# VISION-SJTU/UniDefense

Hardware: AMD Instinct MI355X
Metric: images/sec fwd+bwd (256x256, EffNet-b4) (higher is better)
Workload: dtype f32

## Files before the change

### unidefense_amd/csrc/gemm_p3.hip

```cpp
#include "gemm_internal.h"
#include "ud_common.h"

#include <algorithm>
#include <type_traits>

namespace {

constexpr int NT = 512;
constexpr int BK = 32;
constexpr int BM = 128, BN = 128;
constexpr int PLANE_IMG = 128 * 64;

template <int PREC> struct Cfg {
    static constexpr int NPL = PREC;
    static constexpr int OP_IMG = NPL * PLANE_IMG;
    static constexpr int STAGE = 2 * OP_IMG;
    static constexpr int NSTAGE = PREC == 3 ? 3 : 4;
    static constexpr int PT = 4 * NPL;
    static constexpr int NTERM = PREC == 3 ? 6 : PREC == 2 ? 3 : 1;
};

typedef __bf16 bf16x8 __attribute__((ext_vector_type(8)));
typedef _Float16 f16x8 __attribute__((ext_vector_type(8)));
typedef short s16x4 __attribute__((ext_vector_type(4)));
// ... 294 lines not shown
                    for (int r = 0; r < 16; ++r) {
                        const double v = (double)acc[i][j][r];
                        s1 += v;
                        s2 += v * v;
                    }
                s1 += __shfl_xor(s1, 32, 64);
                s2 += __shfl_xor(s2, 32, 64);
                const int col = n0 + wn * 64 + j * 32 + l31;
                if (half == 0 && col < dN) {
                    unsafeAtomicAdd(stat_sum + slot + col, s1);
                    unsafeAtomicAdd(stat_sumsq + slot + col, s2);
                }
            }
        }
        auto store_all = [&](auto mode_c, auto inside_c) {
            constexpr int MODE = decltype(mode_c)::value;
            constexpr bool INSIDE = decltype(inside_c)::value;
#pragma unroll
            for (int i = 0; i < 2; ++i) {
#pragma unroll
                for (int j = 0; j < 2; ++j) {
                    const int col = n0 + wn * 64 + j * 32 + l31;
                    const long off0 = (long)(m0 + wm * 64 + i * 32 + 4 * half) * ldc + col;
                    float* pc = Cp + off0;
#pragma unroll
                    for (int r = 0; r < 16; ++r) {
                        const int dr = (r & 3) + 8 * (r >> 2);
                        if (INSIDE || (m0 + wm * 64 + i * 32 + 4 * half + dr < dM && col < dN)) {
                            const float v = acc[i][j][r];
                            if constexpr (MODE >= 4) {
                                _Float16* p = reinterpret_cast<_Float16*>(Cp) + off0 + (long)dr * ldc;
                                *p = (_Float16)(MODE == 4 ? v : v + (float)*p);
                            } else {
                                float* p = pc + (long)dr * ldc;
                                if constexpr (MODE == 0) *p = v;
                                else if constexpr (MODE == 1) *p += v;
                                else atomicAdd(p, v);
                            }
                        }
                    }
                }
            }
        };
        const bool inside = m0 + BM <= dM && n0 + BN <= dN;
        if (PREC == 1 && c_half) {
            if (inside) {
                if (ep == 0) store_all(integral_constant<int, 4>{}, T{});
                else store_all(integral_constant<int, 5>{}, T{});
            } else {
                if (ep == 0) store_all(integral_constant<int, 4>{}, F{});
                else store_all(integral_constant<int, 5>{}, F{});
            }
        } else if (inside) {
            if (ep == 0) store_all(integral_constant<int, 0>{}, T{});
            else if (ep == 1) store_all(integral_constant<int, 1>{}, T{});
            else store_all(integral_constant<int, 2>{}, T{});
        } else {
            if (ep == 0) store_all(integral_constant<int, 0>{}, F{});
            else if (ep == 1) store_all(integral_constant<int, 1>{}, F{});
            else store_all(integral_constant<int, 2>{}, F{});
        }
    };

    if constexpr (!SK) {
        int tile_m = bx % tiles_m, tile_n = bx / tiles_m;
        if (d.tile_cfg & 0x200) {
            const int GM = (d.tile_cfg >> 12) & 15 ? (d.tile_cfg >> 12) & 15 : 4;
            const int Tn = tiles_m * tiles_n, q = Tn >> 3, r = Tn & 7, x = bx & 7;
            const int o = x * q + (x < r ? x : r) + (bx >> 3);
            const int per_group = GM * tiles_n, g = o / per_group, first_m = g * GM;
            const int gm = min(GM, tiles_m - first_m), in = o - g * per_group;
            tile_n = in / gm;
            tile_m = first_m + in - tile_n * gm;
        }
        const int split = by;
        const int kt_per = (kt_total + d.split_k - 1) / d.split_k;
        const int kt0 = split * kt_per;
        const int nkt = min(kt_per, kt_total - kt0);
        segment(tile_m, tile_n, kt0, nkt, d.out_mode == 3 ? 0 : d.out_mode,
                d.C + (d.out_mode == 3 ? (long)split * d.slice_stride : 0L), true);
    } else {
        const int G = gx, b = bx;
        const int g = (b & 7) * (G >> 3) + (b >> 3);
        const long U = (long)tiles_m * tiles_n * kt_total;
        long u = g * U / G;
        const long u1 = (g + 1) * U / G;
        const int band_tiles = 8 * tiles_m;
        bool first = true;
        while (u < u1) {
            const int tile = (int)(u / kt_total), kt_b = (int)(u - (long)tile * kt_total);
            const int kt_e = (int)min((long)kt_total, kt_b + (u1 - u));
            const int band = tile / band_tiles, in_band = tile - band * band_tiles;
            const int bw = min(8, tiles_n - band * 8);
            const int tile_m = in_band / bw, tile_n = band * 8 + in_band - tile_m * bw;
            const bool whole = kt_b == 0 && kt_e == kt_total;
            segment(tile_m, tile_n, kt_b, kt_e - kt_b, whole ? d.out_mode : 2, d.C, first);
            first = false;
            u += kt_e - kt_b;
        }
    }
}

template <int PREC, int AMODE, int BMODE, bool SK = false>
__global__ __launch_bounds__(NT, 1) void gemm_p3_kernel(const ud_gemm_p3_desc d, int tiles_m, int tiles_n) {
    using CF = Cfg<PREC>;
    __shared__ __attribute__((aligned(1024))) char L[CF::NSTAGE * CF::STAGE];
    p3_body<PREC, AMODE, BMODE, SK>(d, tiles_m, tiles_n, L, (int)blockIdx.x, (int)blockIdx.y, (int)gridDim.x);
}

template <int PREC, int A0 = 0, int B0 = 1, int A1 = 1, int B1 = 1>
__global__ __launch_bounds__(NT, 1) void gemm_p3_pair_kernel(const ud_gemm_p3_desc d0, int tm0, int tn0, int n0,
                                                              const ud_gemm_p3_desc d1, int tm1, int tn1) {
    using CF = Cfg<PREC>;
    __shared__ __attribute__((aligned(1024))) char L[CF::NSTAGE * CF::STAGE];
    const int b = (int)blockIdx.x;
    const bool first = b < (n0 < 0 ? -n0 : n0);
    const int l = first ? b : b - (n0 < 0 ? -n0 : n0);
    if (first == (n0 > 0)) {
        const int T = tm0 * tn0;
        p3_body<PREC, A0, B0, false>(d0, tm0, tn0, L, l % T, l / T, T);
    } else {
        const int T = tm1 * tn1;
        p3_body<PREC, A1, B1, false>(d1, tm1, tn1, L, l % T, l / T, T);
    }
}

int num_cus() {
    static const int n = [] {
        int dev = 0, cus = 0;
        if (hipGetDevice(&dev) != hipSuccess ||
            hipDeviceGetAttribute(&cus, hipDeviceAttributeMultiprocessorCount, dev) != hipSuccess || cus < 8)
            cus = 256;
        return cus;
    }();
    return n;
}

template <int PREC, int AMODE, int BMODE>
int launch(const ud_gemm_p3_desc& d, hipStream_t s) {
    const int tiles_m = ud_cdiv(d.M, BM), tiles_n = ud_cdiv(d.N, BN);
    if (d.tile_cfg & 0x800) {
        const long U = (long)tiles_m * tiles_n * (d.K / BK);
        long G = std::min<long>(num_cus(), U / 4);
        G = std::max<long>(8, G / 8 * 8);
        hipLaunchKernelGGL((gemm_p3_kernel<PREC, AMODE, BMODE, true>), dim3((unsigned)G), dim3(NT), 0, s, d, tiles_m, tiles_n);
    } else {
        dim3 grid((unsigned)(tiles_m * tiles_n), (unsigned)d.split_k, 1);
        hipLaunchKernelGGL((gemm_p3_kernel<PREC, AMODE, BMODE>), grid, dim3(NT), 0, s, d, tiles_m, tiles_n);
    }
    UD_LAUNCH_CHECK();
    return 0;
}

__device__ __forceinline__ uint32_t pack_bf16(float x, float y) {
    typedef __bf16 bf16x2 __attribute__((ext_vector_type(2)));
    bf16x2 v = {(__bf16)x, (__bf16)y};
    return __builtin_bit_cast(uint32_t, v);
}
__device__ __forceinline__ void split2(float x, float y, uint32_t& p0, uint32_t& p1, uint32_t& p2) {
    p0 = pack_bf16(x, y);
    const float rx = x - __uint_as_float(p0 << 16), ry = y - __uint_as_float(p0 & 0xffff0000u);
    p1 = pack_bf16(rx, ry);
    const float sx = rx - __uint_as_float(p1 << 16), sy = ry - __uint_as_float(p1 & 0xffff0000u);
    p2 = pack_bf16(sx, sy);
}

typedef uint32_t u32x4 __attribute__((ext_vector_type(4)));
typedef uint32_t u32x2 __attribute__((ext_vector_type(2)));

__global__ __launch_bounds__(256) void split_planes_kernel(const float* __restrict__ x, long R, int C, long ld,
                                                           uint16_t* __restrict__ out, long panel, long plane) {
    const int tid = threadIdx.x;
    const long row = (long)blockIdx.x * 64 + (tid >> 2);
    const int pan = blockIdx.y, c0 = pan * 32 + (tid & 3) * 8;
    if (row >= R) return;
    f32x4 v0 = {0.f, 0.f, 0.f, 0.f}, v1 = {0.f, 0.f, 0.f, 0.f};
    if (c0 + 8 <= C) {
        v0 = *reinterpret_cast<const f32x4*>(x + row * ld + c0);
        v1 = *reinterpret_cast<const f32x4*>(x + row * ld + c0 + 4);
    } else if (c0 + 4 <= C) {
        v0 = *reinterpret_cast<const f32x4*>(x + row * ld + c0);
    }
    uint32_t a[4], b[4], c[4];
    split2(v0[0], v0[1], a[0], b[0], c[0]);
    split2(v0[2], v0[3], a[1], b[1], c[1]);
    split2(v1[0], v1[1], a[2], b[2], c[2]);
    split2(v1[2], v1[3], a[3], b[3], c[3]);
    const u32x4 p0 = {a[0], a[1], a[2], a[3]}, p1 = {b[0], b[1], b[2], b[3]}, p2 = {c[0], c[1], c[2], c[3]};
    uint16_t* o = out + (long)pan * panel + row * 32 + (tid & 3) * 8;
    *reinterpret_cast<u32x4*>(o) = p0;
    *reinterpret_cast<u32x4*>(o + plane) = p1;
    *reinterpret_cast<u32x4*>(o + 2 * plane) = p2;
}

typedef _Float16 f16x2 __attribute__((ext_vector_type(2)));
__device__ __forceinline__ void split2h(float x, float y, uint32_t& h0, uint32_t& h1) {
    const f16x2 a = {(_Float16)x, (_Float16)y};
    h0 = __builtin_bit_cast(uint32_t, a);
    const f16x2 b = {(_Float16)((x - (float)a[0]) * 2048.f), (_Float16)((y - (float)a[1]) * 2048.f)};
    h1 = __builtin_bit_cast(uint32_t, b);
}

constexpr int H2_MAXQ = 16;

__global__ __launch_bounds__(256) void split_h2_rows_kernel(const float* __restrict__ x, long R, int C, long ld,
                                                            uint16_t* __restrict__ out, long panel, long plane,
                                                            float* __restrict__ inv_scale) {
    const int lane = threadIdx.x & 63;
    const long row = (long)blockIdx.x * 4 + (threadIdx.x >> 6);
    if (row >= R) return;
    const int nq = C >> 2;
    const f32x4* xr = reinterpret_cast<const f32x4*>(x + row * ld);
    f32x4 v[H2_MAXQ];
    float m = 0.f;
#pragma unroll
    for (int i = 0; i < H2_MAXQ; ++i) {
        const int q = lane + 64 * i;
        v[i] = q < nq ? xr[q] : f32x4{0.f, 0.f, 0.f, 0.f};
        m = fmaxf(m, fmaxf(fmaxf(fabsf(v[i][0]), fabsf(v[i][1])), fmaxf(fabsf(v[i][2]), fabsf(v[i][3]))));
    }
    m = ud_wave_max(m);
    const int e = (int)(__float_as_uint(m) >> 23) & 0xff;
    int fs = m > 0.f ? 268 - e : 127;
    fs = fs < 1 ? 1 : fs > 254 ? 254 : fs;
    const float s = __uint_as_float((uint32_t)fs << 23), inv = __uint_as_float((uint32_t)(254 - fs) << 23);
    if (lane == 0) inv_scale[row] = inv;
    const int nq_pad = ((C + 31) >> 5) << 3;
#pragma unroll
    for (int i = 0; i < H2_MAXQ; ++i) {
        const int q = lane + 64 * i;
        if (q < nq_pad) {
            uint32_t a0, a1, b0, b1;
            split2h(v[i][0] * s, v[i][1] * s, a0, a1);
            split2h(v[i][2] * s, v[i][3] * s, b0, b1);
            uint16_t* o = out + (long)(q >> 3) * panel + row * 32 + (q & 7) * 4;
            *reinterpret_cast<u32x2*>(o) = u32x2{a0, b0};
            *reinterpret_cast<u32x2*>(o + plane) = u32x2{a1, b1};
        }
    }
}

constexpr int ABSMAX_SLOTS = 256;
__global__ __launch_bounds__(1024) void absmax_kernel(const float* __restrict__ x, long R, int C, long ld, uint32_t* __restrict__ out) {
    __shared__ float red[16];
    const long nq = R * (long)(C >> 2);
    const int cq = C >> 2;
    const long stride = (long)ABSMAX_SLOTS * 1024;
    float m = 0.f;
    auto at = [&](long q) {
        const long r = q / cq;
        return *reinterpret_cast<const f32x4*>(x + r * ld + (q - r * cq) * 4);
    };
    long q = (long)blockIdx.x * 1024 + threadIdx.x;
    for (; q + stride < nq; q += 2 * stride) {
        const f32x4 v = at(q), w = at(q + stride);
        m = fmaxf(m, fmaxf(fmaxf(fabsf(v[0]), fabsf(v[1])), fmaxf(fabsf(v[2]), fabsf(v[3]))));
        m = fmaxf(m, fmaxf(fmaxf(fabsf(w[0]), fabsf(w[1])), fmaxf(fabsf(w[2]), fabsf(w[3]))));
    }
    if (q < nq) {
        const f32x4 v = at(q);
        m = fmaxf(m, fmaxf(fmaxf(fabsf(v[0]), fabsf(v[1])), fmaxf(fabsf(v[2]), fabsf(v[3]))));
    }
    m = ud_wave_max(m);
    if ((threadIdx.x & 63) == 0) red[threadIdx.x >> 6] = m;
    __syncthreads();
    if (threadIdx.x == 0) {
        float t = red[0];
#pragma unroll
        for (int i = 1; i < 16; ++i) t = fmaxf(t, red[i]);
        out[blockIdx.x] = __float_as_uint(t);
    }
}

__device__ __forceinline__ void h2_scale(uint32_t bits, float& s, float& inv) { ud_h2_scale(bits, s, inv); }

__global__ __launch_bounds__(256) void split_h2_tensor_kernel(const float* __restrict__ x, long R, int C, long ld,
                                                              uint16_t* __restrict__ out, long panel, long plane,
                                                              const uint32_t* __restrict__ absmax, float* __restrict__ inv_scale) {
    const int tid = threadIdx.x;
    const long row = (long)blockIdx.x * 64 + (tid >> 2);
    const int pan = blockIdx.y, c0 = pan * 32 + (tid & 3) * 8;
    uint32_t mb = 0;
#pragma unroll
    for (int i = 0; i < ABSMAX_SLOTS / 64; ++i) mb = max(mb, absmax[(tid & 63) + 64 * i]);
#pragma unroll
    for (int o = 32; o > 0; o >>= 1) mb = max(mb, (uint32_t)__shfl_xor((int)mb, o, 64));
    float s, inv;
    h2_scale(mb, s, inv);
    if (blockIdx.x == 0 && blockIdx.y == 0 && tid == 0) *inv_scale = inv;
    if (row >= R) return;
    f32x4 v0 = {0.f, 0.f, 0.f, 0.f}, v1 = {0.f, 0.f, 0.f, 0.f};
    if (c0 + 8 <= C) {
        v0 = *reinterpret_cast<const f32x4*>(x + row * ld + c0);
        v1 = *reinterpret_cast<const f32x4*>(x + row * ld + c0 + 4);
    } else if (c0 + 4 <= C) {
        v0 = *reinterpret_cast<const f32x4*>(x + row * ld + c0);
    }
    uint32_t a[4], b[4];
    split2h(v0[0] * s, v0[1] * s, a[0], b[0]);
    split2h(v0[2] * s, v0[3] * s, a[1], b[1]);
    split2h(v1[0] * s, v1[1] * s, a[2], b[2]);
    split2h(v1[2] * s, v1[3] * s, a[3], b[3]);
    uint16_t* o = out + (long)pan * panel + row * 32 + (tid & 3) * 8;
    *reinterpret_cast<u32x4*>(o) = u32x4{a[0], a[1], a[2], a[3]};
    *reinterpret_cast<u32x4*>(o + plane) = u32x4{b[0], b[1], b[2], b[3]};
}
// ... 102 lines not shown
    float m = 0.f;
    for (long q = (long)bl * 1024 + threadIdx.x; q < nq; q += stride) {
        const long r = q / cq;
        const f32x4 v = *reinterpret_cast<const f32x4*>(it.x + r * it.ld + (q - r * cq) * 4);
        m = fmaxf(m, fmaxf(fmaxf(fabsf(v[0]), fabsf(v[1])), fmaxf(fabsf(v[2]), fabsf(v[3]))));
    }
    m = ud_wave_max(m);
    if ((threadIdx.x & 63) == 0) red[threadIdx.x >> 6] = m;
    __syncthreads();
    if (threadIdx.x == 0) {
        float t = red[0];
#pragma unroll
        for (int k = 1; k < 16; ++k) t = fmaxf(t, red[k]);
        slots[(long)i * ABSMAX_SLOTS + bl] = __float_as_uint(t);
    }
}

__global__ __launch_bounds__(256) void split_h2_multi_kernel(const ud_split_item* __restrict__ items, int n,
                                                             const uint32_t* __restrict__ slots) {
    const int i = item_of_block(items, n, blockIdx.x, true);
    const ud_split_item it = items[i];
    const int bl = blockIdx.x - it.split_block0;
    const int pan = bl / it.split_bx, bx = bl - pan * it.split_bx;
    const int tid = threadIdx.x;
    const long row = (long)bx * 64 + (tid >> 2);
    const int c0 = pan * 32 + (tid & 3) * 8;
    const uint32_t* absmax = slots + (long)i * ABSMAX_SLOTS;
    uint32_t mb = 0;
#pragma unroll
    for (int k = 0; k < ABSMAX_SLOTS / 64; ++k) mb = max(mb, absmax[(tid & 63) + 64 * k]);
#pragma unroll
    for (int o = 32; o > 0; o >>= 1) mb = max(mb, (uint32_t)__shfl_xor((int)mb, o, 64));
    float s, inv;
    h2_scale(mb, s, inv);
    if (bl == 0 && tid == 0) *it.inv_scale = inv;
    if (row >= it.R) return;
    f32x4 v0 = {0.f, 0.f, 0.f, 0.f}, v1 = {0.f, 0.f, 0.f, 0.f};
    if (c0 + 8 <= it.C) {
        v0 = *reinterpret_cast<const f32x4*>(it.x + row * it.ld + c0);
        v1 = *reinterpret_cast<const f32x4*>(it.x + row * it.ld + c0 + 4);
    } else if (c0 + 4 <= it.C) {
        v0 = *reinterpret_cast<const f32x4*>(it.x + row * it.ld + c0);
    }
    uint32_t a[4], b[4];
    split2h(v0[0] * s, v0[1] * s, a[0], b[0]);
    split2h(v0[2] * s, v0[3] * s, a[1], b[1]);
    split2h(v1[0] * s, v1[1] * s, a[2], b[2]);
    split2h(v1[2] * s, v1[3] * s, a[3], b[3]);
    uint16_t* o = it.out + (long)pan * it.panel + row * 32 + (tid & 3) * 8;
    *reinterpret_cast<u32x4*>(o) = u32x4{a[0], a[1], a[2], a[3]};
    *reinterpret_cast<u32x4*>(o + it.plane) = u32x4{b[0], b[1], b[2], b[3]};
}

}

extern "C" int ud_split_planes_h2t_multi(const ud_split_item* items_dev, int n, uint32_t* slots, int amax_blocks_total,
                                         int split_blocks_total, ud_stream_t stream) {
    if (!items_dev || !slots || n < 1 || amax_blocks_total < n || split_blocks_total < n) return UD_EINVAL;
    hipStream_t s = (hipStream_t)stream;
    hipLaunchKernelGGL(absmax_multi_kernel, dim3((unsigned)amax_blocks_total), dim3(1024), 0, s, items_dev, n, slots);
    hipLaunchKernelGGL(split_h2_multi_kernel, dim3((unsigned)split_blocks_total), dim3(256), 0, s, items_dev, n, slots);
    UD_LAUNCH_CHECK();
    return 0;
}

extern "C" int ud_im2col_planes(const float* x, const ud_conv_geom* g, uint16_t* planes, long panel_stride, long plane_stride,
                                const uint32_t* absmax, float* inv_scale, ud_stream_t stream) {
    if (!x || !g || !planes || !absmax || !inv_scale || g->transposed || g->Cin < 32 || g->Cin % 32 || g->N < 1 || g->Hin < 1 ||
        g->Win < 1 || g->Hout < 1 || g->Wout < 1 || g->KH < 1 || g->KW < 1 || g->stride < 1)
        return UD_EINVAL;
    const long M = (long)g->N * g->Hout * g->Wout, Kc = (long)g->KH * g->KW * g->Cin;
    if (panel_stride < M * 32 || panel_stride % 8 || plane_stride % 8 || plane_stride < (Kc / 32) * panel_stride) return UD_EINVAL;
    dim3 grid((unsigned)ud_cdiv(M, 64), (unsigned)(Kc / 32));
    hipLaunchKernelGGL(im2col_planes_kernel, grid, dim3(256), 0, (hipStream_t)stream, x, *g, planes, panel_stride, plane_stride,
                       absmax, inv_scale);
    UD_LAUNCH_CHECK();
    return 0;
}

extern "C" int ud_col2im(const float* dcol, const ud_conv_geom* g, float* dx, ud_stream_t stream) {
    if (!dcol || !g || !dx || g->transposed || g->Cin % 4 || g->stride < 1) return UD_EINVAL;
    const long total = (long)g->N * g->Hin * g->Win * (g->Cin / 4);
    long blocks = (total + 255) / 256;
    if (blocks > 16384) blocks = 16384;
    hipLaunchKernelGGL(col2im_kernel, dim3((unsigned)blocks), dim3(256), 0, (hipStream_t)stream, dcol, *g, dx);
    UD_LAUNCH_CHECK();
    return 0;
}

extern "C" int ud_absmax(const float* x, long R, int C, long ld, uint32_t* out, ud_stream_t stream) {
    if (!x || !out || R <= 0 || C <= 0 || C % 4 != 0 || ld % 4 != 0 || ld < C) return UD_EINVAL;
    hipLaunchKernelGGL(absmax_kernel, dim3(ABSMAX_SLOTS), dim3(1024), 0, (hipStream_t)stream, x, R, C, ld, out);
    UD_LAUNCH_CHECK();
    return 0;
}

extern "C" int ud_split_planes_h2t(const float* x, long R, int C, long ld, uint16_t* planes, long panel_stride,
                                   long plane_stride, const uint32_t* absmax, float* inv_scale, ud_stream_t stream) {
    if (!x || !planes || !absmax || !inv_scale || R <= 0 || C <= 0 || C % 4 != 0 || ld % 4 != 0 || ld < C ||
        panel_stride < R * 32 || panel_stride % 8 != 0 || plane_stride % 8 != 0 ||
        plane_stride < (long)ud_cdiv(C, 32) * panel_stride)
        return UD_EINVAL;
    dim3 grid((unsigned)ud_cdiv(R, 64), (unsigned)ud_cdiv(C, 32));
    hipLaunchKernelGGL(split_h2_tensor_kernel, grid, dim3(256), 0, (hipStream_t)stream, x, R, C, ld, planes, panel_stride,
                       plane_stride, absmax, inv_scale);
    UD_LAUNCH_CHECK();
    return 0;
}

extern "C" int ud_planes_from_half(const void* x, long R, int C, long ld, uint16_t* planes, long panel_stride, float* inv_scale,
                                   ud_stream_t stream) {
    if (!x || !planes || !inv_scale || R < 1 || C < 8 || C % 8 || ld < C || ld % 8 || panel_stride < 32 * R || panel_stride % 8 ||
        ((uintptr_t)x & 15))
        return UD_EINVAL;
    dim3 grid((unsigned)ud_cdiv(R, 64), (unsigned)ud_cdiv(C, 32));
    hipLaunchKernelGGL(planes_from_half_kernel, grid, dim3(256), 0, (hipStream_t)stream, (const uint16_t*)x, R, C, ld, planes,
                       panel_stride, inv_scale);
    UD_LAUNCH_CHECK();
    return 0;
}

extern "C" int ud_split_planes(const float* x, long R, int C, long ld, uint16_t* planes, long panel_stride,
                               long plane_stride, ud_stream_t stream) {
    if (!x || !planes || R <= 0 || C <= 0 || C % 4 != 0 || ld % 4 != 0 || ld < C || panel_stride < R * 32 ||
        panel_stride % 8 != 0 || plane_stride % 8 != 0 || plane_stride < (long)ud_cdiv(C, 32) * panel_stride)
        return UD_EINVAL;
    dim3 grid((unsigned)ud_cdiv(R, 64), (unsigned)ud_cdiv(C, 32));
    hipLaunchKernelGGL(split_planes_kernel, grid, dim3(256), 0, (hipStream_t)stream, x, R, C, ld, planes, panel_stride,
                       plane_stride);
    UD_LAUNCH_CHECK();
    return 0;
}

extern "C" int ud_split_planes_h2(const float* x, long R, int C, long ld, uint16_t* planes, long panel_stride,
                                  long plane_stride, float* inv_scale, ud_stream_t stream) {
    if (!x || !planes || !inv_scale || R <= 0 || C <= 0 || C % 4 != 0 || C > 256 * H2_MAXQ || ld % 4 != 0 || ld < C ||
        panel_stride < R * 32 || panel_stride % 8 != 0 || plane_stride % 8 != 0 ||
        plane_stride < (long)ud_cdiv(C, 32) * panel_stride)
        return UD_EINVAL;
    hipLaunchKernelGGL(split_h2_rows_kernel, dim3((unsigned)ud_cdiv(R, 4)), dim3(256), 0, (hipStream_t)stream, x, R, C, ld,
                       planes, panel_stride, plane_stride, inv_scale);
    UD_LAUNCH_CHECK();
    return 0;
}

static bool p3_desc_ok(const ud_gemm_p3_desc& d);

extern "C" int ud_gemm_p3_pair(const ud_gemm_p3_desc* nn, const ud_gemm_p3_desc* tn, ud_stream_t stream) {
    if (!nn || !tn || !p3_desc_ok(*nn) || !p3_desc_ok(*tn)) return UD_EINVAL;
    const ud_gemm_p3_desc &d0 = *nn, &d1 = *tn;
    const bool grads = d0.a_mode == 0 && d0.b_mode == 1 && d1.a_mode == 1 && d1.b_mode == 1;
    const bool tailp = d0.a_mode == 0 && d0.b_mode == 0 && d1.a_mode == 0 && d1.b_mode == 0 && d0.prec == 2;
    if ((d0.prec != 2 && d0.prec != 1) || d1.prec != d0.prec || !(grads || tailp)) return UD_EINVAL;
    if ((d0.tile_cfg | d1.tile_cfg) & 0x800) return UD_EINVAL;
    if (d0.stat_sum || d1.stat_sum || d0.out_mode == 3 || d1.out_mode == 3) return UD_EINVAL;
    const int tm0 = ud_cdiv(d0.M, BM), tn0 = ud_cdiv(d0.N, BN), tm1 = ud_cdiv(d1.M, BM), tn1 = ud_cdiv(d1.N, BN);
    const long n0 = (long)tm0 * tn0 * d0.split_k, n1 = (long)tm1 * tn1 * d1.split_k;
    if (n0 + n1 > 0x7fffffffL) return UD_EINVAL;
    const int nfirst = (d1.tile_cfg & 0x10000) ? -(int)n1 : (int)n0;
    if (tailp)
        hipLaunchKernelGGL((gemm_p3_pair_kernel<2, 0, 0, 0, 0>), dim3((unsigned)(n0 + n1)), dim3(NT), 0, (hipStream_t)stream, d0, tm0,
                           tn0, nfirst, d1, tm1, tn1);
    else if (d0.prec == 1)
        hipLaunchKernelGGL((gemm_p3_pair_kernel<1>), dim3((unsigned)(n0 + n1)), dim3(NT), 0, (hipStream_t)stream, d0, tm0, tn0,
                           nfirst, d1, tm1, tn1);
    else
        hipLaunchKernelGGL((gemm_p3_pair_kernel<2>), dim3((unsigned)(n0 + n1)), dim3(NT), 0, (hipStream_t)stream, d0, tm0, tn0,
                           nfirst, d1, tm1, tn1);
    UD_LAUNCH_CHECK();
    return 0;
}

static bool p3_desc_ok(const ud_gemm_p3_desc& d) {
    if (!d.A || !d.B || !d.C || d.M <= 0 || d.N <= 0 || d.K <= 0 || d.K % BK != 0 || d.split_k < 1 ||
        d.split_k > d.K / BK || d.out_mode < 0 || d.out_mode > 3 || d.a_mode < 0 || d.a_mode > 1 || d.b_mode < 0 ||
        d.b_mode > 1 || d.a_panel % 8 != 0 || d.b_panel % 8 != 0 || d.a_plane % 8 != 0 || d.b_plane % 8 != 0 ||
        d.a_npanel < 1 || d.b_npanel < 1 || d.prec < 1 || d.prec > 3)
        return false;
    if (d.prec <= 2 && (!d.a_inv_scale || !d.b_inv_scale || d.a_scale_stride < 0 || d.a_scale_stride > 1 ||
                        d.b_scale_stride < 0 || d.b_scale_stride > 1))
        return false;
    if (d.stat_sum && (d.out_mode != 0 || d.split_k != 1 || !d.stat_sumsq || (d.tile_cfg & 0x800))) return false;
    if ((d.tile_cfg & 0x800) && (d.out_mode > 1 || d.split_k != 1)) return false;
    if (d.out_mode == 3 && d.slice_stride < (long)d.M * d.ldc) return false;
    if (d.c_half && (d.prec != 1 || d.out_mode > 1 || d.split_k != 1 || (d.tile_cfg & 0x800))) return false;
    return true;
}

extern "C" int ud_gemm_p3(const ud_gemm_p3_desc* dp, ud_stream_t stream) {
    if (!dp) return UD_EINVAL;
    const ud_gemm_p3_desc& d = *dp;
    if (!p3_desc_ok(d)) return UD_EINVAL;
    hipStream_t s = (hipStream_t)stream;
    if (d.prec == 1) {
        if (d.a_mode == 0 && d.b_mode == 0) return launch<1, 0, 0>(d, s);
        if (d.a_mode == 0 && d.b_mode == 1) return launch<1, 0, 1>(d, s);
        if (d.a_mode == 1 && d.b_mode == 1) return launch<1, 1, 1>(d, s);
        return UD_EINVAL;
    }
    if (d.prec == 2) {
        if (d.a_mode == 0 && d.b_mode == 0) return launch<2, 0, 0>(d, s);
        if (d.a_mode == 0 && d.b_mode == 1) return launch<2, 0, 1>(d, s);
        if (d.a_mode == 1 && d.b_mode == 1) return launch<2, 1, 1>(d, s);
        return UD_EINVAL;
    }
    if (d.a_mode == 0 && d.b_mode == 0) return launch<3, 0, 0>(d, s);
    if (d.a_mode == 0 && d.b_mode == 1) return launch<3, 0, 1>(d, s);
    if (d.a_mode == 1 && d.b_mode == 1) return launch<3, 1, 1>(d, s);
    if (d.a_mode == 1 && d.b_mode == 0) return launch<3, 1, 0>(d, s);
    return UD_EINVAL;
}
```

### unidefense_amd/kernels.py

```python
import ctypes as C
import math
import os

import torch

from . import lib as _lib
from .config import cfg as CFG
from .devmem import Scratch, ZeroPool
from .lib import ConvGeom, GemmDesc, GemmP3Desc

_call = _lib.call
_const, _rows = _lib.const, _lib.const_rows

GEMM_PROFILE = None


def _stream():
    return C.c_void_p(torch.cuda.current_stream().cuda_stream)


def _p(t):
    if t is None:
        return None
    return C.c_void_p(t.data_ptr())
# ... 570 lines not shown
            e1.record()
        e1.synchronize()
        cur.wait_stream(s)
        return e0.elapsed_time(e1) / (2 * n)
    except Exception:
        torch.cuda.synchronize()
        e0.record()
        for _ in range(n):
            fn()
        e1.record()
        e1.synchronize()
        return e0.elapsed_time(e1) / n


def _tuned_plan(kind, M, N, K, launch, baseline, extra_if_split=None, no_split=False):
    kind = kind if isinstance(kind, str) else "/".join(str(v) for v in kind)
    key = (kind, M, N, K, extra_if_split is not None, _call("ud_gemm_get_path"))
    if key in _TUNED:
        return _TUNED[key]
    if not CFG.gemm_tune or torch.cuda.is_current_stream_capturing() or min(M, N, K) < _X3_MINDIM:
        return None
    best_t, best = _time_launches(baseline), None
    extra = _time_launches(extra_if_split) if extra_if_split is not None else 0.0
    for cfg, split in _tune_candidates(M, N, K):
        if no_split and split > 1:
            continue
        t = _time_launches(lambda: launch(cfg, split)) + (extra if split > 1 else 0.0)
        if t < 0.97 * best_t:
            best_t, best = t, (cfg, split)
    _TUNED[key] = best
    _tune_cache_save()
    return best


def _model_plan_launch(a, w, out, M, N, K, lda, ldb, b_mode, acc):
    plan = _tail_plan(M, N, K)
    if plan is not None:
        m1, split = plan
        if not acc:
            out = empty((M, N), a)
        _gemm(a, w, out, m1, N, K, lda, ldb, N, 0, b_mode, 1 if acc else 0)
        tail = out[m1:]
        if not acc:
            tail.zero_()
        _gemm(a[m1:], w, tail, M - m1, N, K, lda, ldb, N, 0, b_mode, 2, split)
        return out
    split = _fwd_split(M, N, K)
    if split > 1:
        if not acc:
            out = split_out((M, N), a)
        return _gemm(a, w, out, M, N, K, lda, ldb, N, 0, b_mode, 2, split)
    if not acc:
        out = empty((M, N), a)
    return _gemm(a, w, out, M, N, K, lda, ldb, N, 0, b_mode, 1 if acc else 0)


def _tuned_launch(kind, a, w, out, M, N, K, lda, ldb, a_mode, b_mode, acc, stats, model, out_dtype=torch.float32):
    tmp = []
    kind = kind if out_dtype == torch.float32 and a.dtype == torch.float32 else kind + "/h"

    def scratch():
        if not tmp:
            tmp.append(empty((M, N), a, out_dtype))
        return tmp[0]
    sacc = []

    def stats_pass():
        if not sacc:
            sacc.append(torch.zeros(2 * N, dtype=torch.float64, device=a.device))
        colstats(scratch(), sacc[0])
    tuned = _tuned_plan(kind, M, N, K,
                        lambda cfg, split: _gemm(a, w, scratch(), M, N, K, lda, ldb, N, a_mode, b_mode,
                                                 2 if split > 1 else 0, split, cfg=cfg),
                        lambda: model(scratch()),
                        stats_pass if stats is not None else None, no_split=out_dtype != torch.float32)
    if tuned is None:
        return None
    cfg, split = tuned
    if split == 1:
        if not acc:
            out = empty((M, N), a, out_dtype)
        return _gemm(a, w, out, M, N, K, lda, ldb, N, a_mode, b_mode, 1 if acc else 0, stats=stats, cfg=cfg)
    if not acc:
        out = split_out((M, N), a)
    r = _gemm(a, w, out, M, N, K, lda, ldb, N, a_mode, b_mode, 2, split, cfg=cfg)
    return (r, False) if stats is not None else r


def gemm_nt(a, w, out=None, accumulate=False, stats=None):
    half = _act(a)
    _chk(w)
    M, K = a.shape
    N = w.shape[0]
    assert w.shape[1] == K
    if half:
        if out is None:
            r = _tuned_launch("nt", a, w, None, M, N, K, K, K, 0, 0, False, stats,
                              lambda scr: _gemm(a, w, scr, M, N, K, K, K, N, 0, 0, 0), out_dtype=a.dtype)
            if r is not None:
                return r
            out = empty((M, N), a, a.dtype)
        return _gemm(a, w, out, M, N, K, K, K, N, 0, 0, 1 if accumulate else 0, stats=stats)
    if out is None:
        r = _tuned_launch("nt", a, w, None, M, N, K, K, K, 0, 0, False, stats,
                          lambda scr: _model_plan_launch(a, w, scr, M, N, K, K, K, 0, True))
        if r is not None:
            return r
    if stats is not None:
        assert out is None and not accumulate
        if _tail_plan(M, N, K) is None and _fwd_split(M, N, K) <= 1:
            return _gemm(a, w, empty((M, N), a), M, N, K, K, K, N, 0, 0, 0, stats=stats)
        return _model_plan_launch(a, w, None, M, N, K, K, K, 0, False), False
    if out is None:
        return _model_plan_launch(a, w, None, M, N, K, K, K, 0, False)
    return _gemm(a, w, out, M, N, K, K, K, N, 0, 0, 1 if accumulate else 0)


def gemm_nn(a, w, out=None, accumulate=False):
    half = _act(a, out)
    _chk(w)
    M, K = a.shape
    N = w.shape[1]
    assert w.shape[0] == K
    if half:
        acc = out is not None and accumulate
        if out is None or acc:
            r = _tuned_launch("nn", a, w, out, M, N, K, K, N, 0, 1, acc, None,
                              lambda scr: _gemm(a, w, scr, M, N, K, K, N, N, 0, 1, 0), out_dtype=a.dtype)
            if r is not None:
                return r
        if out is None:
            out = empty((M, N), a, a.dtype)
        return _gemm(a, w, out, M, N, K, K, N, N, 0, 1, 1 if acc else 0)
    if out is None or accumulate:
        acc = out is not None
        r = _tuned_launch("nn", a, w, out, M, N, K, K, N, 0, 1, acc, None,
                          lambda scr: _model_plan_launch(a, w, scr, M, N, K, K, N, 1, True))
        if r is not None:
            return r
        return _model_plan_launch(a, w, out, M, N, K, K, N, 1, acc)
    return _gemm(a, w, out, M, N, K, K, N, N, 0, 1, 0)


_P2_MIN = (1024, 512)
_P2_SPLITS = (2, 3, 4, 6, 8)
_P2_TN_SPLITS = (1, 2, 3, 4, 6, 8, 12, 16, 24, 32, 48, 64, 96, 128, 192, 256)
_P2_MODES = {"nt": (0, 0), "nn": (0, 1), "tn": (1, 1)}


def _p2_shape_ok(M, N, K):
    return M % 32 == 0 and K % 4 == 0 and N % 4 == 0 and min(N, K) >= 64 and M >= 128


def _p2_plans(kind, M, N, K):
    tiles = -(-M // 128) * -(-N // 128)
    out = []
    if kind == "tn":
        for s_ in _P2_TN_SPLITS:
            if (s_ == 1 or K // 32 // s_ >= 4) and 64 <= tiles * s_ <= 2048:
                out.append(("split", s_) if s_ > 1 else ("plain",))
    else:
        out.append(("plain",))
        for s_ in _P2_SPLITS:
            if K // 32 // s_ >= 4 and tiles * s_ <= 2048:
                out.append(("split", s_))
        tp = _tail_plan(M, N, K)
        if tp is not None:
            out.append(("tail", tp[0], tp[1]))
        if kind == "nt" and not CFG.deterministic:
            out += [("tailp", m1, s_) for m1, s_ in _tailp_plans(M, N, K)]
    if not CFG.deterministic:
        out.append(("sk",))
    return out or [("plain",)]


def _tailp_plans(M, N, K):
    if M < 256 or N < 128 or K < 256:
        return []
    mt, nt = -(-M // 128), -(-N // 128)
    full, tail = divmod(mt * nt, 256)
    if full < 1 or tail == 0:
        return []
    out = []
    for extra in (0, 1):
        rows_tail = -(-tail // nt) + extra
        tail_tiles = rows_tail * nt
        if rows_tail >= mt or tail_tiles > 224:
            continue
        for s_ in sorted({max(2, min(16, 256 // tail_tiles)), max(2, min(16, 512 // tail_tiles))}):
            if K // 32 // s_ >= 4:
                out.append(((mt - rows_tail) * 128, s_))
    return out


def _p2_run(kind, plan, ap, bp, M, N, K, like, stats=None, out=None):
    am, bm = _P2_MODES[kind]
    Kp = -(-K // 32) * 32
    how = plan[0]
    if how == "tailp" and GEMM_PROFILE is not None:
        how = "tail"
    acc = out is not None
    assert not (acc and stats is not None)
    odt = torch.float16 if (like.dtype == torch.float16 and kind != "tn") else torch.float32
    assert odt == torch.float32 or how == "plain"
    if how == "plain":
        return _gemm_p3(ap, bp, out if acc else empty((M, N), like, odt), M, N, Kp, am, bm, 1 if acc else 0, 1, stats=stats)
    res = None
    if how == "split":
        res = _gemm_p3(ap, bp, out if acc else split_out((M, N), like), M, N, Kp, am, bm, 2, int(plan[1]))
    elif how == "sk":
        res = _gemm_p3(ap, bp, out if acc else zeros((M, N), like), M, N, Kp, am, bm, 1 if acc else 0, 1, cfg=0x800)
    elif how == "tailp":
        m1, s_ = int(plan[1]), int(plan[2])
        assert kind == "nt"
        res = out if acc else empty((M, N), like)
        tail = res[m1:]
        if not acc:
            tail.zero_()
        d0 = _p3_desc(ap, bp, res, m1, N, Kp, am, bm, 1 if acc else 0, 1)
        d1 = _p3_desc(ap, bp, tail, M - m1, N, Kp, am, bm, 2, s_, a_row0=m1)
        _call("ud_gemm_p3_pair", C.byref(d0), C.byref(d1), _stream())
    else:
        m1, s_ = int(plan[1]), int(plan[2])
        res = out if acc else empty((M, N), like)
        _gemm_p3(ap, bp, res, m1, N, Kp, am, bm, 1 if acc else 0, 1)
        tail = res[m1:]
        if not acc:
            if CFG.deterministic:
                tail._ud_fresh = True
            else:
                tail.zero_()
        _gemm_p3(ap, bp, tail, M - m1, N, Kp, am, bm, 2, s_, a_row0=m1)
    return (res, False) if stats is not None else res


def _p2_default_plan(kind, M, N, K):
    tiles = -(-M // 128) * -(-N // 128)
    if kind == "tn":
        s_ = max(1, min(256 // tiles if tiles <= 256 else 1, K // 32 // 4))
        return ("split", s_) if s_ > 1 else ("plain",)
    full, rem = divmod(tiles, 256)
    if full >= 1 and 0 < rem <= 64:
        tp = _tail_plan(M, N, K)
        if tp is not None:
            return ("tail", tp[0], tp[1])
        if not CFG.deterministic:
            return ("sk",)
    if tiles < 128 and K >= 1024:
        return ("split", min(4, max(2, 256 // tiles)))
    return ("plain",)


_HALF_LIKE = {}


def _half_like(t):
    h = _HALF_LIKE.get(t.device)
    if h is None:
        h = _HALF_LIKE[t.device] = torch.empty(0, dtype=torch.float16, device=t.device)
    return h


def spectral_takes_plane_half(M, N, Kd):
    return _p1_plans_for(M, N, Kd) is not None


def rfft2_plane_half_ok(x):
    if not (x.dtype == torch.float16 and CFG.spectral_p2 != "off"):
        return False
    N, S, _, Cc = x.shape
    return S in (8, 16, 32, 12, 24, 48) and (2 * Cc) % 32 == 0 and not _fft_two_pass("rfft_ex", S, 1)


def rfft2_ex_plane_half(x, scale, w_interior=1.0, bn=None, want_act=False, gate_alpha=None, gate_mode=0, update=False,
                        gate_acc=None, dw_wt=None, dw_k=0):
    _act(x)
    N, S, S2, Cc = x.shape
    assert S == S2 and x.dtype == torch.float16
    pl = Planes(N * S * (S // 2 + 1), 2 * Cc, x, 1, False)
    act = torch.empty_like(x) if (want_act and bn is not None) else None
    ggrad = empty((), x) if gate_acc is not None else None
    spat = torch.empty_like(x) if dw_k else None
    _call("ud_rfft2_ex_plane_half", _p(x), _p(pl.buf), pl.panel, _p(pl.inv), N, S, Cc, float(scale), float(w_interior),
          C.byref(bn.ref(update)) if bn is not None else None, _p(act), _p(gate_alpha), int(gate_mode),
          _pd(gate_acc) if gate_acc is not None else None, _p(ggrad), _p(dw_wt), _p(spat), int(dw_k), _stream())
    out = (pl, act, ggrad) if gate_acc is not None else (pl, act)
    return out + (spat,) if dw_k else out


def planes_from_half(x2):
    R, Cc = x2.shape
    assert x2.is_cuda and x2.dtype == torch.float16 and x2.stride(1) == 1 and x2.stride(0) % 8 == 0
    pl = Planes(R, Cc, x2, 1, False)
    _call("ud_planes_from_half", _p(x2), R, Cc, x2.stride(0), _p(pl.buf), pl.panel, _p(pl.inv), _stream())
    return pl


_P1_MIN = (1024, 128)


def _p1_plans_for(M, N, Kd):
    if not (CFG.spectral_p2 != "off" and _call("ud_gemm_get_path") == 3 and _p2_shape_ok(M, N, Kd) and
            Kd % 8 == 0 and N % 8 == 0 and M >= _P1_MIN[0] and min(N, Kd) >= _P1_MIN[1]):
        return None
    return {"nt": ("plain",), "nn": ("plain",), "tn": _p2_default_plan("tn", N, Kd, M)}


class SpectralCtx:
    __slots__ = ("plans", "x", "w", "dy", "M", "N", "K")


def _p2_block_plans(x2, w2, want_stats=False):
    M, Kd = x2.shape
    if x2.dtype != torch.float32:
        return _p1_plans_for(M, w2.shape[0], Kd) if (x2.dtype == torch.float16 and w2.dtype == torch.float32) else None
    return _p2_plans_for(M, w2.shape[0], Kd, want_stats, w2, x2)


def _p2_plans_for(M, N, Kd, want_stats, w2, x2, tune=True, force=False):
    mode = CFG.spectral_p2
    if (mode == "off" or w2.dtype != torch.float32 or not _p2_shape_ok(M, N, Kd) or
            _call("ud_gemm_get_path") not in (0, 2)):
        return None
    key = ("p2c", M, N, Kd, bool(CFG.deterministic), mode == "on", bool(want_stats))
    plans = _TUNED.get(key, "?")
    if plans is None and force:
        plans = "?"
        tune = False
    if plans == "?":
        if tune and x2 is not None and CFG.gemm_tune and not torch.cuda.is_current_stream_capturing():
            plans = _p2_tune(key, x2, w2, M, N, Kd, mode == "on", want_stats)
        elif mode == "on" or force or (M >= _P2_MIN[0] and min(N, Kd) >= _P2_MIN[1]):
            plans = [("plain",) if want_stats else _p2_default_plan("nt", M, N, Kd), _p2_default_plan("nn", M, Kd, N),
                     _p2_default_plan("tn", N, Kd, M)]
        else:
            plans = None
    if plans is None:
        return None
    return {"nt": tuple(plans[0]), "nn": tuple(plans[1]), "tn": tuple(plans[2])}


def spectral_fwd(x2, w2, stats=None, x_absmax=None, force=False):
    ctx = SpectralCtx()
    ctx.N = w2.shape[0]
    ctx.dy = None
    if isinstance(x2, Planes):
        ctx.M, ctx.K = x2.R, x2.C
        if x2.prec == 1:
            ctx.plans = _p1_plans_for(ctx.M, ctx.N, ctx.K)
            like = _half_like(w2)
        else:
            ctx.plans = _p2_plans_for(ctx.M, ctx.N, ctx.K, stats is not None, w2, None, force=force)
            like = w2
        assert ctx.plans is not None
        ctx.x, ctx.w = x2, weight_planes(w2)
        return _p2_run("nt", ctx.plans["nt"], ctx.x, ctx.w, ctx.M, ctx.N, ctx.K, like, stats=stats), ctx
    ctx.M, ctx.K = x2.shape
    ctx.plans = _p2_block_plans(x2, w2, stats is not None)
    if ctx.plans is None:
        ctx.x, ctx.w = x2, w2
        return gemm_nt(x2, w2, stats=stats), ctx
    if x2.dtype == torch.float16:
        ctx.x, ctx.w = planes_from_half(x2), weight_planes(w2)
    else:
        ctx.x, ctx.w = split_planes(x2, prec=2, absmax=x_absmax), weight_planes(w2)
    return _p2_run("nt", ctx.plans["nt"], ctx.x, ctx.w, ctx.M, ctx.N, ctx.K, x2, stats=stats), ctx


def spectral_takes_planes(M, N, Kd, w2, want_stats=False):
    return _p2_plans_for(M, N, Kd, want_stats, w2, None, tune=False) is not None


def _spectral_dy(ctx, dy2, absmax=None):
    if ctx.dy is None:
        ctx.dy = planes_from_half(dy2) if dy2.dtype == torch.float16 else split_planes(dy2, prec=2, absmax=absmax)
    return ctx.dy


def spectral_dgrad(ctx, dy2, out=None, dy_absmax=None):
    if ctx.plans is None:
        return gemm_nn(dy2, ctx.w, out=out, accumulate=out is not None)
    return _p2_run("nn", ctx.plans["nn"], _spectral_dy(ctx, dy2, dy_absmax), ctx.w, ctx.M, ctx.K, ctx.N, dy2, out=out)


def spectral_wgrad(ctx, dy2, dy_absmax=None):
    if ctx.plans is None:
        return gemm_tn(dy2, ctx.x)
    return _p2_run("tn", ctx.plans["tn"], _spectral_dy(ctx, dy2, dy_absmax), ctx.x, ctx.N, ctx.K, ctx.M, dy2)


def _p2_tune(key, x2, w2, M, N, Kd, forced, want_stats=False):
    dy2 = torch.randn(M, N, device=x2.device)
    acc = torch.zeros(2 * N, dtype=torch.float64, device=x2.device) if want_stats else None

    def fwd_x3():
        r = gemm_nt(x2, w2, stats=acc)
        if want_stats and not r[1]:
            colstats(r[0], acc)
    t_x3 = _time_launches(lambda: (fwd_x3(), gemm_nn(dy2, w2), gemm_tn(dy2, x2)))
    xp, wp, dp = split_planes(x2, prec=2), split_planes(w2, prec=2), split_planes(dy2, prec=2)
    t_p2 = _time_launches(lambda: (split_planes(x2, xp), split_planes(dy2, dp), split_planes(w2, wp)))
    t_stats = _time_launches(lambda: colstats(dy2, acc)) if want_stats else 0.0
    plans = []
    for kind, (a, b, m, n, k) in (("nt", (xp, wp, M, N, Kd)), ("nn", (dp, wp, M, Kd, N)), ("tn", (dp, xp, N, Kd, M))):
        best, best_t = None, 1e30
        for plan in _p2_plans(kind, m, n, k):
            st = acc if (kind == "nt" and want_stats) else None
            t = _time_launches(lambda: _p2_run(kind, plan, a, b, m, n, k, x2, stats=st))
            if st is not None and plan[0] != "plain":
                t += t_stats
            if t < best_t:
                best, best_t = plan, t
        plans.append(list(best))
        t_p2 += best_t
    res = plans if (forced or t_p2 < 0.97 * t_x3) else None
    _TUNED[key] = res
    _tune_cache_save()
    return res


_WG_SPLIT_MAXT = 512
_WG_SPLIT_TARGET = 768
_WG_SPLIT_ROWS = 256


def _pick_split(tiles, K):
    if tiles >= _WG_SPLIT_MAXT or K < 512:
        return 1
    s = min(max(1, K // _WG_SPLIT_ROWS), -(-_WG_SPLIT_TARGET // tiles))
    return max(1, min(s, 1024))


_TILE_CFGS = ((128, 128, 1.00), (128, 64, 0.93), (256, 32, 1.10), (32, 256, 1.10), (64, 128, 0.93))


_FWD_SPLIT_T = 224
_FWD_SPLIT_K = 512
_FWD_SPLIT_MINK = 256
_FWD_SPLIT_WGS = 320


def _fwd_split(M, N, K):
    t = _tiles(M, N)
    if t >= _FWD_SPLIT_T or K < _FWD_SPLIT_K:
        return 1
    return max(1, min(K // _FWD_SPLIT_MINK, -(-_FWD_SPLIT_WGS // t)))


_X3_MINDIM = 16


def _tiles(M, N):
    best, best_tiles = None, 1
    for bm, bn, pen in _TILE_CFGS:
        t = -(-M // bm) * -(-N // bn)
        cost = -(-t // 256) * bm * bn * pen
        if best is None or cost < best:
            best, best_tiles = cost, t
    return best_tiles


def gemm_tn(a, b):
    _act(a, b)
    K, M = a.shape
    N = b.shape[1]
    assert b.shape[0] == K
    split = _pick_split(_tiles(M, N), K)
    r = _tuned_launch("tn", a, b, None, M, N, K, M, N, 1, 1, False, None,
                      lambda scr: _gemm(a, b, scr, M, N, K, M, N, N, 1, 1, 2 if split > 1 else 0, split))
    if r is not None:
        return r
    if split > 1:
        out = split_out((M, N), a)
        return _gemm(a, b, out, M, N, K, M, N, N, 1, 1, 2, split)
    out = empty((M, N), a)
    return _gemm(a, b, out, M, N, K, M, N, N, 1, 1, 0, 1)


def conv_geom(N, Hin, Win, Cin, Hout, Wout, KH, KW, stride, pad_t, pad_l, transposed=0):
    g = ConvGeom()
    g.N, g.Hin, g.Win, g.Cin, g.Hout, g.Wout = N, Hin, Win, Cin, Hout, Wout
    g.KH, g.KW, g.stride, g.pad_t, g.pad_l, g.transposed = KH, KW, stride, pad_t, pad_l, transposed
    return g


_CONV_SPLITK = True


_CONV_SMALL = True
_CONV_SMALL_MIN_M = 262144
_CONV_SMALL_OK = {}


def _conv_small_supported(Ci, Co, KH, KW):
    key = (Ci, Co, KH, KW)
    if key not in _CONV_SMALL_OK:
        _CONV_SMALL_OK[key] = _call("ud_conv_small_supported", Ci, Co, KH, KW) == 1
    return _CONV_SMALL_OK[key]


_CONV_SMALL_WS = Scratch(torch.float32)
_CONV_SMALL_WGRAD_OK = {}


def _conv_small_wgrad_supported(Ci, Ma, KH, KW):
    key = (Ci, Ma, KH, KW)
    if key not in _CONV_SMALL_WGRAD_OK:
        _CONV_SMALL_WGRAD_OK[key] = _call("ud_conv_small_wgrad_supported", Ci, Ma, KH, KW) == 1
    return _CONV_SMALL_WGRAD_OK[key]


_CONV_MFMA = True
_CONV_MFMA_MIN_M = 16384
_CONV_MFMA_SHAPES = frozenset({(20, 20, 0), (40, 20, 0), (40, 40, 0), (20, 40, 0), (80, 40, 0), (80, 80, 0), (40, 80, 0),
                               (20, 20, 1), (40, 40, 1), (80, 80, 1), (20, 20, 2)})
_CONV_MFMA_OK = {}


def _conv_mfma_mode(g):
    return int(_lib.load().ud_conv_mfma_mode(C.byref(g)))


def _conv_mfma_takes(g, Co, M, *tensors):
    if not _CONV_MFMA or M < _CONV_MFMA_MIN_M:
        return False
    key = (g.Cin, Co, _conv_mfma_mode(g))
    if key[2] < 0 or (_CONV_MFMA_SHAPES is not None and key not in _CONV_MFMA_SHAPES):
        return False
    if key not in _CONV_MFMA_OK:
        _CONV_MFMA_OK[key] = _call("ud_conv_mfma_supported", *key) == 1
    return _CONV_MFMA_OK[key] and all(t.dtype == torch.float32 and t.data_ptr() % 16 == 0 for t in tensors)


_CONV_MFMA_WGRAD_SHAPES = frozenset()
_CONV_MFMA_WGRAD_OK = {}
_CONV_MFMA_WS = Scratch(torch.float32)


def _conv_mfma_wgrad_takes(g, Ma, M, *tensors):
    if not _CONV_MFMA or M < _CONV_MFMA_MIN_M:
        return False
    key = (g.Cin, Ma, _conv_mfma_mode(g))
    if key[2] not in (0, 2) or (_CONV_MFMA_WGRAD_SHAPES is not None and key not in _CONV_MFMA_WGRAD_SHAPES):
        return False
    if key not in _CONV_MFMA_WGRAD_OK:
        _CONV_MFMA_WGRAD_OK[key] = _call("ud_conv_mfma_wgrad_supported", *key) == 1
    return _CONV_MFMA_WGRAD_OK[key] and all(t.dtype == torch.float32 and t.data_ptr() % 16 == 0 for t in tensors)


def conv_gather_nt(x, wmat, g):
    _chk(x, wmat)
    M = g.N * g.Hout * g.Wout
    K = g.KH * g.KW * g.Cin
    Co = wmat.shape[0]
    assert wmat.shape[1] == K and x.numel() == g.N * g.Hin * g.Win * g.Cin
    if _conv_mfma_takes(g, Co, M, x, wmat):
        out = empty((g.N, g.Hout, g.Wout, Co), x)
        _call("ud_conv_mfma", C.byref(g), _p(x), _p(wmat), _p(out), Co, _stream())
        return out
    if _CONV_SMALL and M >= _CONV_SMALL_MIN_M and _conv_small_supported(g.Cin, Co, g.KH, g.KW):
        out = empty((g.N, g.Hout, g.Wout, Co), x)
        _call("ud_conv_small", C.byref(g), _p(x), _p(wmat), _p(out), Co, _stream())
# ... 2491 lines not shown
```

Measured before the change: 1445.

## Add 64x64 single-wave small-tile GEMM variant for prec-2 autotune plans

```diff
diff --git a/unidefense_amd/csrc/gemm_p3.hip b/unidefense_amd/csrc/gemm_p3.hip
--- a/unidefense_amd/csrc/gemm_p3.hip
+++ b/unidefense_amd/csrc/gemm_p3.hip
@@ -470,6 +470,222 @@
     return 0;
 }
 
+constexpr int SM = 64, SN = 64;
+constexpr int S_OP = SM * 64;
+constexpr int S_STAGE = 4 * S_OP, S_NSTAGE = 1;
+static_assert(2 * S_OP == PLANE_IMG, "A | B interleave: the planes of one operand are PLANE_IMG apart");
+
+typedef unsigned u32x4 __attribute__((ext_vector_type(4)));
+template <int MODE>
+struct SmallTileLoader {
+    const char *g0, *g1;
+    long step, plane;
+    unsigned src, dst;
+    u32x4 r[8];
+
+    __device__ __forceinline__ void init(const uint16_t* X, long panel, long plane_, int npanel, int row0, int lane) {
+        plane = plane_ * 2;
+        if constexpr (MODE == 0) {
+            g0 = g1 = reinterpret_cast<const char*>(X) + (long)row0 * 64;
+            step = panel * 2;
+            src = (unsigned)lane * 16u;
+            dst = (unsigned)((lane >> 2) * 64 + (((lane & 3) ^ ((lane >> 4) & 3)) << 4));
+        } else {
+            g0 = reinterpret_cast<const char*>(X) + (long)min(row0 / 32, npanel - 1) * panel * 2;
+            g1 = reinterpret_cast<const char*>(X) + (long)min(row0 / 32 + 1, npanel - 1) * panel * 2;
+            step = BK * 64;
+            src = dst = (unsigned)lane * 16u;
+        }
+    }
+    __device__ __forceinline__ void load(int t) {
+#pragma unroll
+        for (int pl = 0; pl < 2; ++pl)
+#pragma unroll
+            for (int i = 0; i < 4; ++i) {
+                const char* p = MODE == 0 ? g0 + i * 1024 : (i < 2 ? g0 : g1) + (i & 1) * 1024;
+                r[pl * 4 + i] = *reinterpret_cast<const u32x4*>(p + (long)t * step + pl * plane + src);
+            }
+    }
+    __device__ __forceinline__ void store(lds_char* img) const {
+#pragma unroll
+        for (int pl = 0; pl < 2; ++pl)
+#pragma unroll
+            for (int i = 0; i < 4; ++i)
+                *reinterpret_cast<__attribute__((address_space(3))) u32x4*>(img + pl * PLANE_IMG + i * 1024 + dst) = r[pl * 4 + i];
+    }
+};
+
+template <int BMODE>
+__global__ __launch_bounds__(64, 2) void gemm_p3_small_kernel(const ud_gemm_p3_desc d, int tiles_n) {
+    __shared__ __attribute__((aligned(1024))) char L[S_NSTAGE * S_STAGE];
+    using std::integral_constant;
+    const int lane = threadIdx.x;
+    const int l31 = lane & 31, half = lane >> 5;
+    int o = (int)blockIdx.x;
+    if (d.tile_cfg & 0x200) {
+        const int Tn = (int)gridDim.x, q = Tn >> 3, r = Tn & 7, x = o & 7;
+        o = x * q + (x < r ? x : r) + (o >> 3);
+    }
+    const int tile_m = o / tiles_n, tile_n = o - tile_m * tiles_n;
+    const int m0 = tile_m * SM, n0 = tile_n * SN;
+    const int nkt = d.K / BK;
+    const int dM = d.M, dN = d.N;
+    const long ldc = d.ldc;
+    double* const stat_sum = d.stat_sum;
+    double* const stat_sumsq = d.stat_sumsq;
+    const float* __restrict__ as = d.a_inv_scale;
+    const float* __restrict__ bs = d.b_inv_scale;
+    const long ast = d.a_scale_stride, bst = d.b_scale_stride;
+    lds_char* Lp = (lds_char*)L;
+
+    SmallTileLoader<0> la;
+    SmallTileLoader<BMODE> lb;
+    la.init(d.A, d.a_panel, d.a_plane, d.a_npanel, m0, lane);
+    lb.init(d.B, d.b_panel, d.b_plane, d.b_npanel, n0, lane);
+    la.load(0);
+    lb.load(0);
+    float ib[2];
+#pragma unroll
+    for (int j = 0; j < 2; ++j) ib[j] = bs[(long)min(n0 + j * 32 + l31, dN - 1) * bst];
+    const float ia0 = as[0];
+
+    Reader<0> ra;
+    Reader<BMODE> rb;
+    ra.init(lane, 0);
+    rb.init(lane, 0);
+    f32x16 acc[2][2], lo[2][2];
+#pragma unroll
+    for (int i = 0; i < 2; ++i)
+#pragma unroll
+        for (int j = 0; j < 2; ++j)
+#pragma unroll
+            for (int r = 0; r < 16; ++r) {
+                acc[i][j][r] = 0.f;
+                lo[i][j][r] = 0.f;
+            }
+
+    la.store(Lp);
+    lb.store(Lp + S_OP);
+    __syncthreads();
+
+    auto kstep = [&](const Frags<2>& a, const Frags<2>& b) {
+        mma_one<2, 0>(acc, lo, a, b); mma_one<2, 1>(acc, lo, a, b); mma_one<2, 2>(acc, lo, a, b); mma_one<2, 3>(acc, lo, a, b);
+        mma_one<2, 4>(acc, lo, a, b); mma_one<2, 5>(acc, lo, a, b); mma_one<2, 6>(acc, lo, a, b); mma_one<2, 7>(acc, lo, a, b);
+        mma_one<2, 8>(acc, lo, a, b); mma_one<2, 9>(acc, lo, a, b); mma_one<2, 10>(acc, lo, a, b); mma_one<2, 11>(acc, lo, a, b);
+    };
+    for (int t = 0; t < nkt; ++t) {
+        const lds_char* img = Lp + (t % S_NSTAGE) * S_STAGE;
+        const bool more = t + 1 < nkt;
+        if (more) {
+            la.load(t + 1);
+            lb.load(t + 1);
+        }
+        Frags<2> fa, fb;
+        ra.template read<0>(img, fa);
+        rb.template read<0>(img + S_OP, fb);
+        kstep(fa, fb);
+        ra.template read<1>(img, fa);
+        rb.template read<1>(img + S_OP, fb);
+        kstep(fa, fb);
+        if (more) {
+            if constexpr (S_NSTAGE == 1) __syncthreads();
+            lds_char* nxt = Lp + ((t + 1) % S_NSTAGE) * S_STAGE;
+            la.store(nxt);
+            lb.store(nxt + S_OP);
+        }
+        __syncthreads();
+    }
+
+    float ia[2][16];
+    if (ast == 0) {
+        const float a0 = ia0;
+#pragma unroll
+        for (int i = 0; i < 2; ++i)
+#pragma unroll
+            for (int r = 0; r < 16; ++r) ia[i][r] = a0;
+    } else {
+#pragma unroll
+        for (int i = 0; i < 2; ++i)
+#pragma unroll
+            for (int r = 0; r < 16; ++r) ia[i][r] = as[min(m0 + i * 32 + (r & 3) + 8 * (r >> 2) + 4 * half, dM - 1)];
+    }
+#pragma unroll
+    for (int j = 0; j < 2; ++j) {
+        const bool cok = n0 + j * 32 + l31 < dN;
+#pragma unroll
+        for (int i = 0; i < 2; ++i)
+#pragma unroll
+            for (int r = 0; r < 16; ++r) {
+                const int row = m0 + i * 32 + (r & 3) + 8 * (r >> 2) + 4 * half;
+                float v = acc[i][j][r];
+                v += 0x1p-11f * lo[i][j][r];
+                v *= ia[i][r] * ib[j];
+                acc[i][j][r] = (cok && row < dM) ? v : 0.f;
+            }
+    }
+    if (stat_sum) {
+        const long slot = (dM > 64 * BM) ? (long)((m0 / BM) & 63) * dN : 0;
+#pragma unroll
+        for (int j = 0; j < 2; ++j) {
+            double s1 = 0.0, s2 = 0.0;
+#pragma unroll
+            for (int i = 0; i < 2; ++i)
+#pragma unroll
+                for (int r = 0; r < 16; ++r) {
+                    const double v = (double)acc[i][j][r];
+                    s1 += v;
+                    s2 += v * v;
+                }
+            s1 += __shfl_xor(s1, 32, 64);
+            s2 += __shfl_xor(s2, 32, 64);
+            const int col = n0 + j * 32 + l31;
+            if (half == 0 && col < dN) {
+                unsafeAtomicAdd(stat_sum + slot + col, s1);
+                unsafeAtomicAdd(stat_sumsq + slot + col, s2);
+            }
+        }
+    }
+    auto store_all = [&](auto add_c, auto inside_c) {
+        constexpr bool ADD = decltype(add_c)::value;
+        constexpr bool INSIDE = decltype(inside_c)::value;
+#pragma unroll
+        for (int i = 0; i < 2; ++i)
+#pragma unroll
+            for (int j = 0; j < 2; ++j) {
+                const int col = n0 + j * 32 + l31;
+                float* pc = d.C + (long)(m0 + i * 32 + 4 * half) * ldc + col;
+#pragma unroll
+                for (int r = 0; r < 16; ++r) {
+                    const int dr = (r & 3) + 8 * (r >> 2);
+                    if (INSIDE || (m0 + i * 32 + 4 * half + dr < dM && col < dN)) {
+                        float* p = pc + (long)dr * ldc;
+                        if constexpr (ADD) *p += acc[i][j][r];
+                        else *p = acc[i][j][r];
+                    }
+                }
+            }
+    };
+    using T = std::true_type;
+    using F = std::false_type;
+    const bool inside = m0 + SM <= dM && n0 + SN <= dN;
+    if (d.out_mode == 0) {
+        if (inside) store_all(F{}, T{});
+        else store_all(F{}, F{});
+    } else {
+        if (inside) store_all(T{}, T{});
+        else store_all(T{}, F{});
+    }
+}
+
+template <int BMODE>
+int launch_small(const ud_gemm_p3_desc& d, hipStream_t s) {
+    const long tiles_m = ud_cdiv(d.M, SM), tiles_n = ud_cdiv(d.N, SN);
+    if (tiles_m * tiles_n > 0x7fffffffL) return UD_EINVAL;
+    hipLaunchKernelGGL((gemm_p3_small_kernel<BMODE>), dim3((unsigned)(tiles_m * tiles_n)), dim3(64), 0, s, d, (int)tiles_n);
+    UD_LAUNCH_CHECK();
+    return 0;
+}
+
 __device__ __forceinline__ uint32_t pack_bf16(float x, float y) {
     typedef __bf16 bf16x2 __attribute__((ext_vector_type(2)));
     bf16x2 v = {(__bf16)x, (__bf16)y};
@@ -878,7 +1094,7 @@
     const bool grads = d0.a_mode == 0 && d0.b_mode == 1 && d1.a_mode == 1 && d1.b_mode == 1;
     const bool tailp = d0.a_mode == 0 && d0.b_mode == 0 && d1.a_mode == 0 && d1.b_mode == 0 && d0.prec == 2;
     if ((d0.prec != 2 && d0.prec != 1) || d1.prec != d0.prec || !(grads || tailp)) return UD_EINVAL;
-    if ((d0.tile_cfg | d1.tile_cfg) & 0x800) return UD_EINVAL;
+    if ((d0.tile_cfg | d1.tile_cfg) & (0x800 | 0x400)) return UD_EINVAL;
     if (d0.stat_sum || d1.stat_sum || d0.out_mode == 3 || d1.out_mode == 3) return UD_EINVAL;
     const int tm0 = ud_cdiv(d0.M, BM), tn0 = ud_cdiv(d0.N, BN), tm1 = ud_cdiv(d1.M, BM), tn1 = ud_cdiv(d1.N, BN);
     const long n0 = (long)tm0 * tn0 * d0.split_k, n1 = (long)tm1 * tn1 * d1.split_k;
@@ -910,6 +1126,8 @@
     if ((d.tile_cfg & 0x800) && (d.out_mode > 1 || d.split_k != 1)) return false;
     if (d.out_mode == 3 && d.slice_stride < (long)d.M * d.ldc) return false;
     if (d.c_half && (d.prec != 1 || d.out_mode > 1 || d.split_k != 1 || (d.tile_cfg & 0x800))) return false;
+    if ((d.tile_cfg & 0x400) && (d.prec != 2 || d.c_half || d.a_mode != 0 || d.out_mode > 1 || d.split_k != 1 || (d.tile_cfg & 0x800)))
+        return false;
     return true;
 }
 
@@ -925,6 +1143,7 @@
         return UD_EINVAL;
     }
     if (d.prec == 2) {
+        if (d.tile_cfg & 0x400) return d.b_mode == 0 ? launch_small<0>(d, s) : launch_small<1>(d, s);
         if (d.a_mode == 0 && d.b_mode == 0) return launch<2, 0, 0>(d, s);
         if (d.a_mode == 0 && d.b_mode == 1) return launch<2, 0, 1>(d, s);
         if (d.a_mode == 1 && d.b_mode == 1) return launch<2, 1, 1>(d, s);
diff --git a/unidefense_amd/kernels.py b/unidefense_amd/kernels.py
--- a/unidefense_amd/kernels.py
+++ b/unidefense_amd/kernels.py
@@ -746,6 +746,9 @@
     return M % 32 == 0 and K % 4 == 0 and N % 4 == 0 and min(N, K) >= 64 and M >= 128
 
 
+_P2_SMALL_MAX_TILES = 1024
+
+
 def _p2_plans(kind, M, N, K):
     tiles = -(-M // 128) * -(-N // 128)
     out = []
@@ -755,6 +758,8 @@
                 out.append(("split", s_) if s_ > 1 else ("plain",))
     else:
         out.append(("plain",))
+        if tiles <= _P2_SMALL_MAX_TILES:
+            out.append(("small",))
         for s_ in _P2_SPLITS:
             if K // 32 // s_ >= 4 and tiles * s_ <= 2048:
                 out.append(("split", s_))
@@ -799,6 +804,9 @@
     assert odt == torch.float32 or how == "plain"
     if how == "plain":
         return _gemm_p3(ap, bp, out if acc else empty((M, N), like, odt), M, N, Kp, am, bm, 1 if acc else 0, 1, stats=stats)
+    if how == "small":
+        assert kind != "tn"
+        return _gemm_p3(ap, bp, out if acc else empty((M, N), like), M, N, Kp, am, bm, 1 if acc else 0, 1, stats=stats, cfg=0x400)
     res = None
     if how == "split":
         res = _gemm_p3(ap, bp, out if acc else split_out((M, N), like), M, N, Kp, am, bm, 2, int(plan[1]))
@@ -1001,7 +1009,7 @@
         for plan in _p2_plans(kind, m, n, k):
             st = acc if (kind == "nt" and want_stats) else None
             t = _time_launches(lambda: _p2_run(kind, plan, a, b, m, n, k, x2, stats=st))
-            if st is not None and plan[0] != "plain":
+            if st is not None and plan[0] not in ("plain", "small"):
                 t += t_stats
             if t < best_t:
                 best, best_t = plan, t
```

Result: no change. 1447, median of 4 (+0.1%).
